# ranjanbalappa-nykaa/recommendations

Measured on AMD Instinct MI355X. Metric: training samples/sec (LTHM fwd+bwd) at 1/2/4/8 MI355X; embedding HBM GB/s, higher is better.
Workload: dtype bf16; 1 GPU; LTHM C2: item KShift P=1000000 D=32 K=16, 32 cat x 1000000 KShift D=32 K=8, T=128, d=256, 4 layers, H=4, 6 lookahead heads; global_batch=4096, per_gpu_batch=4096, seq_len=128, activation_checkpointing=False, distinct_batches=4, item_lookup=inline, parallelism=dp1

## Files before the change

### recommendations_amd/csrc/loss.hip

```cpp
#include "mfma.hpp"

#include <algorithm>
#include <cstdlib>

namespace lthm {

constexpr int DE = 128;

__device__ __forceinline__ int swz(int row) {
  const int h = (row >> 3) & 1;
  return ((((row & 7) << 1) + (h << 3)) & 15) | h;
}
__device__ __forceinline__ int ks_off256(int row, int ch) { return row * 256 + ((ch ^ swz(row)) << 4); }

template <typename TX>
__global__ __launch_bounds__(256) void rownorm_k(const TX* __restrict__ x, int64_t rows, int D, bf16_t* __restrict__ out,
                                                 float* __restrict__ norms, const uint8_t* __restrict__ mask,
                                                 int64_t mgroup, int64_t mstride) {
  const int lane = threadIdx.x & 63;
  for (int64_t r = (int64_t)blockIdx.x * 4 + (threadIdx.x >> 6); r < rows; r += (int64_t)gridDim.x * 4) {
    float v[4];
    float ss = 0.f;
#pragma unroll
    for (int i = 0; i < 4; ++i) {
// ... 1565 lines not shown
      v2 += __popcll(__ballot(ok));
    }
    if (lane == 0) { V[b] = v; V2[b] = v2; }
  }
  __syncthreads();
  const int per = (Bm + 255) / 256;
  const int r0 = min(tid * per, Bm), r1 = min(r0 + per, Bm);
  for (int pass = 0; pass < (phys ? 2 : 1); ++pass) {
    int* A = pass ? V2 : V;
    int run = 0;
    for (int b = r0; b < r1; ++b) run += A[b];
    scan[tid] = run;
    __syncthreads();
    for (int o = 1; o < 256; o <<= 1) {
      const int t = tid >= o ? scan[tid - o] : 0;
      __syncthreads();
      scan[tid] += t;
      __syncthreads();
    }
    const int total = scan[255];
    int k = scan[tid] - run;
    __syncthreads();
    for (int b = r0; b < r1; ++b) {
      const int c = A[b];
      A[b] = k;
      k += c;
    }
    if (tid == 0) A[Bm] = total;
    __syncthreads();
  }
  const int N = V[Bm];
  int* cs = a.vcs + (int64_t)mb * (a.mbs + 1);
  for (int b = tid; b <= Bm; b += 256) cs[b] = V[b];
  if (tid == 0) {
    a.vm[mb] = N;
    if (phys) a.vnp[mb] = V2[Bm];
  }
  int* cmap = a.vcmap + (int64_t)mb * a.mbs * T;
  int* pidx = a.vpidx + (int64_t)mb * a.mbs * T;
  const int L = g.L;
  for (int b = wv; b < Bm; b += 4) {
    const uint8_t* mr = mrow(b);
    int* cm = cmap + (int64_t)b * T;
    wave_compact(T, V[b], lane, [&](int tp) { return tp >= off && mr[tp] == 0; },
                 [&](int k, int tp) { a.vridx[base + k] = b * L + tp - off; cm[tp] = k; },
                 [&](int tp) { cm[tp] = -1; });
    if (phys)
      wave_compact(T, V2[b], lane, [&](int tp) { return mr[tp] == 0; },
                   [&](int k, int tp) { pidx[k] = b * T + tp; }, [&](int) {});
  }
  int u = 0;
  for (int b = tid; b < Bm; b += 256) {
    const int vb = V[b + 1] - V[b];
    u += (N - vb > 0) ? vb : 0;
  }
  const int U = (int)block_dsum((double)u, red);
  const float wr = U > 0 ? loss_scale / (float)U : 0.f;
  for (int r = tid; r < a.n_max; r += 256) {
    float wvv = 0.f;
    if (r < g.n) {
      const int b = seq_of(g, r);
      wvv = (!pad_of(a, g, r) && N - (V[b + 1] - V[b]) > 0) ? wr : 0.f;
    }
    wout[base + r] = wvv;
  }
  const int per_row = DE / 4;
  const int64_t cnt = (int64_t)Bm * (T + 1) * per_row;
  for (int64_t i = tid; i < cnt; i += 256) {
    const int row = (int)(i / per_row), c4 = (int)(i - (int64_t)row * per_row);
    const int b = row / (T + 1), t = row - b * (T + 1);
    if (t < L && mrow(b)[t + off] == 0) continue;
    const int64_t o = (((g.b0 + b) * (T + 1) + t) * a.NH + a.head) * DE + c4 * 4;
    if (a.y_dtype == LTHM_BF16) *reinterpret_cast<uint2*>(a.dy + o) = uint2{0u, 0u};
    else *reinterpret_cast<float4*>((float*)a.dy + o) = float4{0.f, 0.f, 0.f, 0.f};
  }
}

template <typename TY>
__global__ __launch_bounds__(256) void cl_vgather_k(ClArgs a0) {
  const ClArgs a = head_args(a0, blockIdx.z);
  const int mb = blockIdx.y;
  const Geo g = geo(a, mb);
  const int m = a.vm[mb];
  const int64_t base = (int64_t)mb * a.n_max;
  const int sub = threadIdx.x & 15;
  const int step = gridDim.x * 32;
  for (int i0 = blockIdx.x * 32 + (threadIdx.x >> 4); i0 < m; i0 += step) {
    int rr[2];
    u32x4 ov[2], iv[2];
    float yv[2][8];
#pragma unroll
    for (int u = 0; u < 2; ++u) rr[u] = a.vridx[base + min(i0 + 16 * u, m - 1)];
#pragma unroll
    for (int u = 0; u < 2; ++u) {
      if (a.vnorm_out) {
        const int b = rr[u] / g.L, t = rr[u] - b * g.L;
        const int64_t ro = ((g.b0 + b) * (a.T + 1) + t) * a.NH + a.head;
        ld8(reinterpret_cast<const TY*>(a.y_raw) + ro * DE + sub * 8, yv[u]);
      } else {
        ov[u] = *reinterpret_cast<const u32x4*>(out_row(a, g, rr[u]) + sub * 8);
      }
      iv[u] = *reinterpret_cast<const u32x4*>(in_row(a, g, rr[u]) + sub * 8);
    }
#pragma unroll
    for (int u = 0; u < 2; ++u) {
      const int i = i0 + 16 * u;
      if (a.vnorm_out) {
        float ss = 0.f;
#pragma unroll
        for (int k = 0; k < 8; ++k) ss += yv[u][k] * yv[u][k];
        const float nrm = sqrtf(group16_sum(ss));
        const float den = fmaxf(nrm, 1e-12f);
        float o[8];
#pragma unroll
        for (int k = 0; k < 8; ++k) o[k] = yv[u][k] / den;
        ov[u] = u32x4{pack_bf16x2(o[0], o[1]), pack_bf16x2(o[2], o[3]), pack_bf16x2(o[4], o[5]), pack_bf16x2(o[6], o[7])};
        if (i < m && sub == 0) {
          const int b = rr[u] / g.L, t = rr[u] - b * g.L;
          a.vnorm_out[((g.b0 + b) * (a.T + 1) + t) * a.NH + a.head] = nrm;
        }
      }
      float acc = 0.f;
#pragma unroll
      for (int k = 0; k < 4; ++k) {
        acc = fmaf(__uint_as_float(ov[u][k] << 16), __uint_as_float(iv[u][k] << 16), acc);
        acc = fmaf(__uint_as_float(ov[u][k] & 0xffff0000u), __uint_as_float(iv[u][k] & 0xffff0000u), acc);
      }
#pragma unroll
      for (int o = 1; o < 16; o <<= 1) acc += __shfl_xor(acc, o, 64);
      if (i < m) {
        *reinterpret_cast<u32x4*>(a.vR + (base + i) * DE + sub * 8) = ov[u];
        *reinterpret_cast<u32x4*>(a.vC + (base + i) * DE + sub * 8) = iv[u];
        if (sub == 0) a.diag[base + rr[u]] = acc / a.tau;
      }
    }
  }
}

__global__ __launch_bounds__(256) void cl_vshift_k(ClArgs a0) {
  const ClArgs a = head_args(a0, blockIdx.z);
  const int mb = blockIdx.y;
  const int m = a.vm[mb];
  const int64_t base = (int64_t)mb * a.n_max;
  for (int i = blockIdx.x * 256 + threadIdx.x; i < m; i += gridDim.x * 256) {
    const int r = a.vridx[base + i];
    const float wv = a.w[base + r];
    a.vsh[base + i] = wv != 0.f ? __log2f(wv) - a.lse[base + r] * LOG2E : -INFINITY;
    a.vw[base + i] = wv;
  }
  if (blockIdx.z != 0) return;
  const Geo g = geo(a, mb);
  const int T = a.T;
  const int per_row = DE / 4;
  const int64_t cnt = (int64_t)g.Bm * T * per_row;
  for (int64_t i = (int64_t)blockIdx.x * 256 + threadIdx.x; i < cnt; i += (int64_t)gridDim.x * 256) {
    const int row = (int)(i / per_row), c4 = (int)(i - (int64_t)row * per_row);
    const int b = row / T, t = row - b * T;
    if (a.mask[(g.b0 + b) * a.mask_stride + t] == 0) continue;
    const int64_t o = ((g.b0 + b) * T + t) * DE + c4 * 4;
    if (a.t_dtype == LTHM_BF16) *reinterpret_cast<uint2*>((bf16_t*)a.dt + o) = uint2{0u, 0u};
    else *reinterpret_cast<float4*>((float*)a.dt + o) = float4{0.f, 0.f, 0.f, 0.f};
  }
}

struct VTile {
  union {
    unsigned char img[CL_NB32][64 * 256];
    float ep[4][32][CL_EPS];
  };
};

struct VCursor {
  const unsigned char* base;
  int row0, lim, ch0;
  __device__ __forceinline__ void init(const bf16_t* base_, int lim_, int w, int lane) {
    base = reinterpret_cast<const unsigned char*>(base_);
    row0 = 16 * w + (lane >> 4);
    lim = lim_;
    ch0 = (lane & 15) ^ (((lane >> 4) & 3) << 2);
  }
  __device__ __forceinline__ void stage(unsigned char* img, int t, int w, int lane) {
#pragma unroll
    for (int k = 0; k < 4; ++k) {
      const int row = 64 * t + row0 + 4 * k;
      const void* src = row < lim ? (const void*)(base + (int64_t)row * 256 + ((ch0 ^ k) << 4))
                                  : (const void*)(cl_zero_row + 16 * (lane & 15));
      glds16(src, img + (16 * w + 4 * k) * 256);
    }
  }
};

struct TileOrder {
  int ts_lo, nspan, nclean, tl, rot;
  __device__ __forceinline__ void init(int spec_lo, int spec_hi, int m, int ntile, bool last_special) {
    ts_lo = spec_lo / 64;
    const int ts_hi = (spec_hi - 1) / 64;
    nspan = ts_hi - ts_lo + 1;
    tl = (last_special && (m & 63) && ntile - 1 > ts_hi) ? ntile - 1 : -1;
    nclean = ntile - nspan - (tl >= 0 ? 1 : 0);
    rot = 0;
  }
  __device__ __forceinline__ int at(int i) const {
    if (i < nclean && rot) {
      i += rot % nclean;
      if (i >= nclean) i -= nclean;
    }
    if (i < ts_lo) return i;
    if (i < nclean) return i + nspan;
    const int j = i - nclean;
    return j < nspan ? ts_lo + j : tl;
  }
};

__device__ __forceinline__ void s_tile32(f32x16 (&acc)[2], const unsigned char* img, const int (&roff)[8],
                                         const bf16x8v (&qf)[8]) {
  acc[0] = f32x16{};
  acc[1] = f32x16{};
  auto rd = [&](int ib, int s) {
    return frag_at(img + ib * 8192 + roff[s]);
  };
  bf16x8v f0 = rd(0, 0), f1 = rd(1, 0);
#pragma unroll
  for (int s = 0; s < 8; ++s) {
    const int sn = s + 1 < 8 ? s + 1 : s;
    const bf16x8v n0 = rd(0, sn), n1 = rd(1, sn);
    acc[0] = mfma32(f0, qf[s], acc[0]);
    acc[1] = mfma32(f1, qf[s], acc[1]);
    f0 = n0;
    f1 = n1;
  }
}

__device__ __forceinline__ void pv_tile32(f32x16 (&dacc)[4], const f32x16& p, int ib, const unsigned char* img,
                                          const int (&toff)[4][2]) {
  const bf16x8v af0 = pack_frag(p, 0), af1 = pack_frag(p, 8);
  const int k0 = 2 * ib * 4096, k1 = (2 * ib + 1) * 4096;
#pragma unroll
  for (int nd = 0; nd < 4; ++nd) {
    dacc[nd] = mfma32(af0, tr_frag32(img, toff[nd][0] + k0, toff[nd][1] + k0), dacc[nd]);
    dacc[nd] = mfma32(af1, tr_frag32(img, toff[nd][0] + k1, toff[nd][1] + k1), dacc[nd]);
  }
}

__global__ __launch_bounds__(256, 2) void cl_fr32v_k(ClArgs a0) {
  constexpr int NW = 4, XR = 32 * NW;
  __shared__ __attribute__((aligned(16))) VTile sh;
  __shared__ float rs_sc[NW][32], rs_w[NW][32], rs_pd[NW][32];
  int z = blockIdx.z, mb = blockIdx.y, xb = blockIdx.x;
  if (a0.xcd_order & 1) {
    const int per = gridDim.x * gridDim.y;
    const int lin = xcd_remap(blockIdx.x + gridDim.x * (blockIdx.y + gridDim.y * blockIdx.z), per * gridDim.z);
    z = lin / per;
    const int bid = lin - z * per;
    mb = bid / gridDim.x;
    xb = bid - mb * gridDim.x;
  }
  const ClArgs a = head_args(a0, z);
  const int m = a.vm[mb];
  const int x0 = xb * XR;
  if (x0 >= m) return;
  const Geo g = geo(a, mb);
  const int tid = threadIdx.x, lane = tid & 63, w = __builtin_amdgcn_readfirstlane(tid >> 6);
  const int r32 = lane & 31, hh = lane >> 5;
  const int64_t base = (int64_t)mb * a.n_max;
  const int* cs = a.vcs + (int64_t)mb * (a.mbs + 1);
  const int* ridx = a.vridx + base;
  int roff[8], toff[4][2];
  frag32_offsets(roff, toff, lane);
  f32x16 dacc[4];
#pragma unroll
  for (int nd = 0; nd < 4; ++nd) dacc[nd] = f32x16{};
  const int x = x0 + 32 * w + r32;
  const bool live = x < m;
  const int r = live ? ridx[x] : 0;
  bf16x8v qf[8];
  {
    const bf16_t* rp = a.vR + (base + (live ? x : 0)) * DE;
#pragma unroll
    for (int s = 0; s < 8; ++s) {
      u32x4 v = {0u, 0u, 0u, 0u};
      if (live) v = *reinterpret_cast<const u32x4*>(rp + 16 * s + 8 * hh);
      qf[s] = __builtin_bit_cast(bf16x8v, v);
    }
  }
  const float it = 1.f / a.tau, c1 = it * LOG2E, csh = -c1;
  const float dg = live ? a.diag[base + r] : 0.f;
  const float thr = rank_threshold(dg, it, a.tau);
  const int xsq = live ? seq_of(g, r) : 0;
  const int xlo = live ? cs[xsq] : -(1 << 30);
  const unsigned xlen = live ? (unsigned)(cs[xsq + 1] - cs[xsq]) : 0u;
  const int rlo = ridx[x0], rhi = ridx[min(x0 + XR, m) - 1];
  const int spec_lo = cs[seq_of(g, rlo)], spec_hi = cs[seq_of(g, rhi) + 1];
  float Z = 0.f;
  int cn = 0, rk = 0;
  const int ntile = (m + 63) / 64;
  TileOrder ord;
  ord.init(spec_lo, spec_hi, m, ntile, true);
  if (a0.xcd_order & 2) ord.rot = xb;
  VCursor cur;
  cur.init(a.vC + base * DE, m, w, lane);
  retire_loads();
  cur.stage(sh.img[0], ord.at(0), w, lane);
  if (ntile > 1) cur.stage(sh.img[1], ord.at(1), w, lane);
  if (ntile > 2) cur.stage(sh.img[2], ord.at(2), w, lane);
  if (ntile > 2) wait_vm<8>();
  else if (ntile > 1) wait_vm<4>();
  else wait_vm<0>();
  __builtin_amdgcn_s_barrier();
  f32x16 sacc[2];
  s_tile32(sacc, sh.img[0], roff, qf);
  auto open_step = [&](int i) {
    if (i + 2 < ntile) wait_vm<4>();
    else wait_vm<0>();
    __builtin_amdgcn_s_barrier();
    if (i + 3 < ntile) cur.stage(sh.img[(i + 3) % CL_NB32], ord.at(i + 3), w, lane);
  };
  for (int i = 0; i < ord.nclean; ++i) {
    open_step(i);
    const unsigned char* img = sh.img[i % CL_NB32];
    const unsigned char* imgn = sh.img[(i + 1) % CL_NB32];
#pragma unroll
    for (int ib = 0; ib < 2; ++ib) {
#pragma unroll
      for (int v = 0; v < 16; ++v) {
        const float sv = sacc[ib][v];
        const float p = __builtin_amdgcn_exp2f(__builtin_fmaf(sv, c1, csh));
        Z += p;
        rk += sv > thr ? 1 : 0;
        sacc[ib][v] = p;
      }
    }
    cn += 32;
    f32x16 snext[2];
    s_tile32(snext, imgn, roff, qf);
    pv_tile32(dacc, sacc[0], 0, img, toff);
    pv_tile32(dacc, sacc[1], 1, img, toff);
    sacc[0] = snext[0];
    sacc[1] = snext[1];
  }
  auto below = [](int k) { return k >= 64 ? ~0ull : (1ull << k) - 1ull; };
  for (int i = ord.nclean; i < ntile; ++i) {
    open_step(i);
    const unsigned char* img = sh.img[i % CL_NB32];
    const unsigned char* imgn = sh.img[(i + 1) % CL_NB32];
    const int y0 = 64 * ord.at(i);
    const int lo = min(max(xlo - y0, 0), 64), hi = min(max(xlo + (int)xlen - y0, 0), 64);
    const int me = min(max(m - y0, 0), 64);
    uint64_t keep = live ? (below(lo) | (below(me) & ~below(hi))) : 0ull;
    keep >>= 4 * hh;
    const uint32_t kw[2] = {(uint32_t)keep, (uint32_t)(keep >> 32)};
    cn += __popc(kw[0] & 0x0F0F0F0Fu) + __popc(kw[1] & 0x0F0F0F0Fu);
#pragma unroll
    for (int ib = 0; ib < 2; ++ib) {
#pragma unroll
      for (int v = 0; v < 16; ++v) {
        const int msk = __builtin_amdgcn_sbfe((int)kw[ib], 8 * (v >> 2) + (v & 3), 1);
        const float sv = __uint_as_float((__float_as_uint(sacc[ib][v]) & msk) | (0xff800000u & ~msk));
        const float p = __builtin_amdgcn_exp2f(__builtin_fmaf(sv, c1, csh));
        Z += p;
        rk += sv > thr ? 1 : 0;
        sacc[ib][v] = p;
      }
    }
    f32x16 snext[2];
    s_tile32(snext, imgn, roff, qf);
    pv_tile32(dacc, sacc[0], 0, img, toff);
    pv_tile32(dacc, sacc[1], 1, img, toff);
    sacc[0] = snext[0];
    sacc[1] = snext[1];
  }
  Z += __shfl_xor(Z, 32, 64);
  cn += __shfl_xor(cn, 32, 64);
  rk += __shfl_xor(rk, 32, 64);
  const float pd = live ? __builtin_amdgcn_exp2f((dg - it) * LOG2E) : 0.f;
  Z += pd;
  cn += live ? 1 : 0;
  const float wx = live ? a.w[base + r] : 0.f;
  if (hh == 0) {
    if (live) {
      a.lse[base + r] = it + __logf(Z);
      a.pos[base + r] = dg;
      a.cnt[base + r] = cn;
      a.rank[base + r] = rk;
    }
    rs_sc[w][r32] = (wx != 0.f && Z > 0.f) ? wx / Z : 0.f;
    rs_w[w][r32] = wx;
    rs_pd[w][r32] = pd;
  }
  __syncthreads();
#pragma unroll
  for (int nd = 0; nd < 4; ++nd)
#pragma unroll
    for (int v = 0; v < 16; ++v) sh.ep[w][8 * (v >> 2) + 4 * hh + (v & 3)][32 * nd + r32] = dacc[nd][v];
  __syncthreads();
  const float gs = 1.f / a.tau;
  const int sub = lane & 15;
#pragma unroll 1
  for (int ps = 0; ps < 8; ++ps) {
    const int rl = 4 * ps + (lane >> 4), xr = x0 + 32 * w + rl;
    const int xc = min(xr, m - 1);
    const int rr = ridx[xc];
    const int b = rr / g.L, t = rr - b * g.L;
    const int64_t ro = ((g.b0 + b) * (a.T + 1) + t) * a.NH + a.head;
    const float sc = rs_sc[w][rl], wr = rs_w[w][rl], pdr = rs_pd[w][rl];
    float inv[8];
    load_vec<bf16_t, 16>(a.vC + (base + xc) * DE + 8 * sub, inv);
    const float4 u0 = *reinterpret_cast<const float4*>(&sh.ep[w][rl][8 * sub]);
    const float4 u1 = *reinterpret_cast<const float4*>(&sh.ep[w][rl][8 * sub + 4]);
    const float uu[8] = {u0.x, u0.y, u0.z, u0.w, u1.x, u1.y, u1.z, u1.w};
    float gv[8];
#pragma unroll
    for (int i = 0; i < 8; ++i) gv[i] = gs * (__builtin_fmaf(pdr, inv[i], uu[i]) * sc - wr * inv[i]);
    normalize_bwd_store(gv, a.y_raw, a.y_dtype, a.y_norm[ro], a.dy, ro * DE + 8 * sub, xr < m);
  }
}

__global__ __launch_bounds__(256, 2) void cl_bwd32v_k(ClArgs a0) {
  constexpr int NW = 4, XR = 32 * NW;
  __shared__ __attribute__((aligned(16))) ClTile32<NW> sh;
  const int per = gridDim.x * gridDim.y;
  const int lin = xcd_remap(blockIdx.x + gridDim.x * blockIdx.y, per);
  const int mb = lin / gridDim.x, xb = lin - mb * gridDim.x;
  const int tid = threadIdx.x, lane = tid & 63, w = __builtin_amdgcn_readfirstlane(tid >> 6);
  const int r32 = lane & 31, hh = lane >> 5;
  const int T = a0.T;
  const int64_t b0 = (int64_t)mb * a0.mbs;
  const int np = a0.vnp[mb];
  const int j0 = xb * XR;
  if (j0 >= np) return;
  const int* pidx = a0.vpidx + (int64_t)mb * a0.mbs * T;
  const int j = j0 + 32 * w + r32;
  const bool pin = j < np;
  const int p = pidx[pin ? j : np - 1];
  const int pb = p / T, pt = p - pb * T;
  int roff[8], toff[4][2];
  frag32_offsets(roff, toff, lane);
  f32x16 dacc[4];
#pragma unroll
  for (int nd = 0; nd < 4; ++nd) dacc[nd] = f32x16{};
  bf16x8v qf[8];
  {
    const bf16_t* rp = a0.in_n + ((b0 + pb) * T + pt) * DE;
#pragma unroll
    for (int s = 0; s < 8; ++s) {
      u32x4 v = {0u, 0u, 0u, 0u};
      if (pin) v = *reinterpret_cast<const u32x4*>(rp + 16 * s + 8 * hh);
      qf[s] = __builtin_bit_cast(bf16x8v, v);
    }
  }
  const int b_lo = pidx[j0] / T, b_hi = pidx[min(j0 + XR, np) - 1] / T;
  const float c1 = LOG2E / a0.tau;
  const int nrun = a0.heads_run;
#pragma unroll 1
  for (int hz = 0; hz < nrun; ++hz) {
    const ClArgs a = head_args(a0, hz);
    const int m = a.vm[mb];
    if (m == 0) continue;
    const int64_t base = (int64_t)mb * a.n_max;
    const int* cs = a.vcs + (int64_t)mb * (a.mbs + 1);
    const int xc = pin ? a.vcmap[(int64_t)mb * a.mbs * T + p] : -1;
    const bool live = xc >= 0;
    const int xlo = cs[pb];
    const unsigned xlen = (unsigned)(cs[pb + 1] - xlo);
    const int spec_lo = cs[b_lo], spec_hi = cs[b_hi + 1];
    const bool wmask = __ballot(!live) != 0ull;
    const float* shv = a.vsh + base;
    const float* wvv = a.vw + base;
    VCursor cur;
    cur.init(a.vR + base * DE, m, w, lane);
    const int ntile = (m + 63) / 64;
    TileOrder ord;
    ord.init(spec_lo, spec_hi, m, ntile, false);
    auto stage = [&](int i) {
      const int buf = i % CL_NB32, y0 = ord.at(i) * 64;
      cur.stage(sh.r.img[buf], ord.at(i), w, lane);
      const bool inr = y0 + lane < m;
      glds4(inr ? shv + y0 + lane : &cl_ninf, sh.r.m0[buf][w]);
      glds4(inr ? wvv + y0 + lane : &cl_zero_f, sh.r.m1[buf][w]);
    };
    constexpr int PT = 6;
    __syncthreads();
    retire_loads();
    stage(0);
    if (ntile > 1) stage(1);
    if (ntile > 2) stage(2);
    auto open_step = [&](int i) {
      if (i + 2 < ntile) wait_vm<2 * PT>();
      else if (i + 1 < ntile) wait_vm<PT>();
      else wait_vm<0>();
      __builtin_amdgcn_s_barrier();
      if (i + 3 < ntile) stage(i + 3);
    };
    for (int i = 0; i < ord.nclean; ++i) {
      open_step(i);
      const int cb = i % CL_NB32;
      const unsigned char* img = sh.r.img[cb];
      f32x16 acc[2];
      s_tile32(acc, img, roff, qf);
#pragma unroll
      for (int ib = 0; ib < 2; ++ib)
#pragma unroll
        for (int qd = 0; qd < 4; ++qd) {
          const float4 ys = *reinterpret_cast<const float4*>(&sh.r.m0[cb][w][32 * ib + 8 * qd + 4 * hh]);
          const float yv[4] = {ys.x, ys.y, ys.z, ys.w};
#pragma unroll
          for (int jj = 0; jj < 4; ++jj)
            acc[ib][4 * qd + jj] = __builtin_amdgcn_exp2f(__builtin_fmaf(acc[ib][4 * qd + jj], c1, yv[jj]));
        }
      if (wmask && !live) {
        acc[0] = f32x16{};
        acc[1] = f32x16{};
      }
      pv_tile32(dacc, acc[0], 0, img, toff);
      pv_tile32(dacc, acc[1], 1, img, toff);
    }
    for (int i = ord.nclean; i < ntile; ++i) {
      open_step(i);
      const int cb = i % CL_NB32;
      const unsigned char* img = sh.r.img[cb];
      f32x16 acc[2];
      s_tile32(acc, img, roff, qf);
      const int y0 = 64 * ord.at(i);
      const int lo = min(max(xlo - y0, 0), 64), hi = min(max(xlo + (int)xlen - y0, 0), 64);
      auto below = [](int k) { return k >= 64 ? ~0ull : (1ull << k) - 1ull; };
      const int dd = xc - y0;
      uint64_t keep = below(lo) | ~below(hi);
      if (live && dd >= 0 && dd < 64) keep |= 1ull << dd;
      keep >>= 4 * hh;
      const uint32_t kw[2] = {(uint32_t)keep, (uint32_t)(keep >> 32)};
      int dx = dd - 4 * hh;
      asm volatile("" : "+v"(dx));
#pragma unroll
      for (int ib = 0; ib < 2; ++ib)
#pragma unroll
        for (int qd = 0; qd < 4; ++qd) {
          const float4 ys = *reinterpret_cast<const float4*>(&sh.r.m0[cb][w][32 * ib + 8 * qd + 4 * hh]);
          const float4 ws = *reinterpret_cast<const float4*>(&sh.r.m1[cb][w][32 * ib + 8 * qd + 4 * hh]);
          const float yv[4] = {ys.x, ys.y, ys.z, ys.w}, wv4[4] = {ws.x, ws.y, ws.z, ws.w};
#pragma unroll
          for (int jj = 0; jj < 4; ++jj) {
            const int v = 4 * qd + jj, cv = 8 * qd + jj;
            const int msk = __builtin_amdgcn_sbfe((int)kw[ib], cv, 1);
            const float sv = __uint_as_float((__float_as_uint(acc[ib][v]) & msk) | (0xff800000u & ~msk));
            const float e = __builtin_amdgcn_exp2f(__builtin_fmaf(sv, c1, yv[jj]));
            const uint32_t dm = 0u - (uint32_t)(dx == 32 * ib + cv);
            acc[ib][v] = e - __uint_as_float(__float_as_uint(wv4[jj]) & dm);
          }
        }
      if (wmask && !live) {
        acc[0] = f32x16{};
        acc[1] = f32x16{};
      }
      pv_tile32(dacc, acc[0], 0, img, toff);
      pv_tile32(dacc, acc[1], 1, img, toff);
    }
  }
  __syncthreads();
#pragma unroll
  for (int nd = 0; nd < 4; ++nd)
#pragma unroll
    for (int v = 0; v < 16; ++v) sh.ep[w][8 * (v >> 2) + 4 * hh + (v & 3)][32 * nd + r32] = dacc[nd][v];
  const float gs = (a0.gscale ? *a0.gscale : 1.f) / a0.tau;
  const int sub = lane & 15;
#pragma unroll 1
  for (int ps = 0; ps < 8; ++ps) {
    const int rl = 4 * ps + (lane >> 4), q = j0 + 32 * w + rl;
    const int pq = pidx[min(q, np - 1)];
    const int64_t ro = b0 * T + pq;
    float gv[8];
    const float4 u0 = *reinterpret_cast<const float4*>(&sh.ep[w][rl][8 * sub]);
    const float4 u1 = *reinterpret_cast<const float4*>(&sh.ep[w][rl][8 * sub + 4]);
    gv[0] = gs * u0.x; gv[1] = gs * u0.y; gv[2] = gs * u0.z; gv[3] = gs * u0.w;
    gv[4] = gs * u1.x; gv[5] = gs * u1.y; gv[6] = gs * u1.z; gv[7] = gs * u1.w;
    normalize_bwd_store(gv, a0.t_raw, a0.t_dtype, a0.t_norm[ro], a0.dt, ro * DE + 8 * sub, q < np);
  }
}

}

using namespace lthm;

static ClArgs cl_args(const lthm_contrastive_desc* d) {
  ClArgs a;
  a.out_n = (const bf16_t*)d->out_n; a.in_n = (const bf16_t*)d->in_n; a.mask = d->mask; a.mask_stride = d->mask_stride;
  a.B = d->B; a.T = d->T; a.NH = d->n_heads; a.head = d->head; a.mbs = d->mb_size; a.n_mb = d->n_mb; a.n_max = d->n_max;
  a.offsets = d->offsets; a.tau = d->tau;
  a.lse = d->lse; a.pos = d->pos; a.cnt = d->cnt; a.rank = d->rank; a.diag = d->diag; a.w = d->w;
  a.gscale = d->gscale;
  a.d_out = d->d_out; a.d_in = d->d_in;
  a.colb = nullptr;
  a.lq = d->logq; a.lq_stride = d->logq_stride; a.lqcol = d->logq_col;
  a.y_raw = (const bf16_t*)d->y_raw; a.y_norm = d->y_norm; a.dy = (bf16_t*)d->dy;
  a.head_stride = d->head_stride;
  a.y_dtype = d->y_dtype;
  a.heads_run = d->heads_run > 1 ? d->heads_run : 1;
  a.t_raw = d->t_raw; a.t_dtype = d->t_dtype; a.t_norm = d->t_norm; a.dt = d->dt;
  a.xcd_order = 0;
  a.vm = nullptr; a.vcs = nullptr; a.vridx = nullptr; a.vsh = nullptr; a.vw = nullptr; a.vcmap = nullptr;
  a.vR = nullptr; a.vC = nullptr; a.vpidx = nullptr; a.vnp = nullptr; a.vnorm_out = nullptr;
  if (d->vc_ws) {
    const VcLayout L = vc_layout(d->n_heads, d->n_mb, d->mb_size, d->T, d->n_max);
    char* b = (char*)d->vc_ws;
    a.vm = (int*)(b + L.m); a.vnp = (int*)(b + L.np); a.vcs = (int*)(b + L.cs); a.vridx = (int*)(b + L.ridx);
    a.vsh = (float*)(b + L.sh); a.vw = (float*)(b + L.w); a.vcmap = (int*)(b + L.cmap); a.vpidx = (int*)(b + L.pidx);
    a.vR = (bf16_t*)(b + L.R); a.vC = (bf16_t*)(b + L.C);
  }
  return a;
}

static int cl_check(const lthm_contrastive_desc* d) {
  if (!d || d->De != DE || d->B <= 0 || d->T <= 0 || d->mb_size <= 0 || d->n_mb <= 0) return 1;
  if ((int64_t)d->mb_size * d->T > d->n_max || d->n_max % 64 != 0) return 1;
  if ((int64_t)d->n_max * d->T >= (1ll << 32)) return 1;
  if (d->head < 0 || d->head >= d->n_heads) return 1;
  if (d->logq && (!d->logq_col || d->logq_stride < d->T)) return 1;
  return 0;
}

static int64_t cl_stats_blocks(int32_t n_max) { return (n_max + CL_SROWS - 1) / CL_SROWS; }

extern "C" int64_t lthm_contrastive_vc_ws_bytes(int64_t B, int32_t T, int32_t n_heads, int32_t mb_size, int32_t n_mb,
                                                int32_t n_max) {
  if (B <= 0 || T <= 0 || n_heads <= 0 || mb_size <= 0 || n_mb <= 0 || n_max <= 0) return -1;
  return vc_layout(n_heads, n_mb, mb_size, T, n_max).total;
}

static bool vc_ok(const lthm_contrastive_desc* d) {
  if (!d->vc_ws) return false;
  if (!d->out_n && !(d->y_raw && d->y_norm)) return false;
  if (d->vc_ws_bytes < vc_layout(d->n_heads, d->n_mb, d->mb_size, d->T, d->n_max).total) return false;
  return d->head == 0 && d->heads_run == d->n_heads && d->head_stride == (int64_t)d->n_mb * d->n_max &&
         d->mb_size <= CL_UMAXB && (int64_t)d->mb_size * d->T <= (1ll << 30);
}

extern "C" int64_t lthm_contrastive_ws_bytes(int32_t n_mb, int32_t n_max, int32_t heads) {
  if (n_mb <= 0 || n_max <= 0 || heads <= 0) return -1;
  const int64_t hm = (int64_t)heads * n_mb;
  return hm * n_max * 4 + ((hm * n_max * 4) % 8) + hm * cl_stats_blocks(n_max) * CL_NPART * 8;
}

template <typename TX>
static void launch_rownorm(const TX* x, int64_t rows, int D, bf16_t* out, float* norms, const uint8_t* mask,
                           int64_t mgroup, int64_t mstride, hipStream_t s) {
  if (D % 8 == 0) {
    const int grid = grid_for(rows, 16, 256 * 8);
    if (D <= 128)
      hipLaunchKernelGGL((rownorm_v8_k<TX, 1>), dim3(grid), dim3(256), 0, s, x, rows, D, out, norms, mask, mgroup, mstride);
    else
      hipLaunchKernelGGL((rownorm_v8_k<TX, 2>), dim3(grid), dim3(256), 0, s, x, rows, D, out, norms, mask, mgroup, mstride);
  } else {
    hipLaunchKernelGGL((rownorm_k<TX>), dim3(grid_for(rows, 4, 256 * 8)), dim3(256), 0, s, x, rows, D, out, norms,
                       mask, mgroup, mstride);
  }
}

template <typename TX>
static void launch_rownorm_bwd(const TX* x, const float* norms, const float* g, int64_t rows, int D, bf16_t* dx_bf,
                               float* dx_f, hipStream_t s) {
  if (D % 8 == 0) {
    const int grid = grid_for(rows, 16, 256 * 8);
    if (D <= 128)
      hipLaunchKernelGGL((rownorm_bwd_v8_k<TX, 1>), dim3(grid), dim3(256), 0, s, x, norms, g, rows, D, dx_bf, dx_f);
    else
      hipLaunchKernelGGL((rownorm_bwd_v8_k<TX, 2>), dim3(grid), dim3(256), 0, s, x, norms, g, rows, D, dx_bf, dx_f);
  } else {
    hipLaunchKernelGGL((rownorm_bwd_k<TX>), dim3(grid_for(rows, 4, 256 * 8)), dim3(256), 0, s, x, norms, g, rows, D,
                       dx_bf, dx_f);
  }
}

extern "C" int lthm_rownorm(const void* x, int32_t x_dtype, int64_t rows, int32_t D, void* out_bf16, float* norms,
                            const uint8_t* row_mask, int64_t mask_group, int64_t mask_stride, void* stream) {
// ... 176 lines not shown
```

Baseline: 109,000 samples/s.

## Process two score tiles per barrier in the loss kernel pipeline

```diff
diff --git a/recommendations_amd/csrc/loss.hip b/recommendations_amd/csrc/loss.hip
--- a/recommendations_amd/csrc/loss.hip
+++ b/recommendations_amd/csrc/loss.hip
@@ -1891,23 +1891,13 @@
   retire_loads();
   cur.stage(sh.img[0], ord.at(0), w, lane);
   if (ntile > 1) cur.stage(sh.img[1], ord.at(1), w, lane);
-  if (ntile > 2) cur.stage(sh.img[2], ord.at(2), w, lane);
-  if (ntile > 2) wait_vm<8>();
-  else if (ntile > 1) wait_vm<4>();
-  else wait_vm<0>();
-  __builtin_amdgcn_s_barrier();
-  f32x16 sacc[2];
-  s_tile32(sacc, sh.img[0], roff, qf);
   auto open_step = [&](int i) {
-    if (i + 2 < ntile) wait_vm<4>();
-    else wait_vm<0>();
+    wait_vm<0>();
     __builtin_amdgcn_s_barrier();
+    if (i + 2 < ntile) cur.stage(sh.img[(i + 2) % CL_NB32], ord.at(i + 2), w, lane);
     if (i + 3 < ntile) cur.stage(sh.img[(i + 3) % CL_NB32], ord.at(i + 3), w, lane);
   };
-  for (int i = 0; i < ord.nclean; ++i) {
-    open_step(i);
-    const unsigned char* img = sh.img[i % CL_NB32];
-    const unsigned char* imgn = sh.img[(i + 1) % CL_NB32];
+  auto elems_clean = [&](f32x16 (&sacc)[2]) {
 #pragma unroll
     for (int ib = 0; ib < 2; ++ib) {
 #pragma unroll
@@ -1920,18 +1910,9 @@
       }
     }
     cn += 32;
-    f32x16 snext[2];
-    s_tile32(snext, imgn, roff, qf);
-    pv_tile32(dacc, sacc[0], 0, img, toff);
-    pv_tile32(dacc, sacc[1], 1, img, toff);
-    sacc[0] = snext[0];
-    sacc[1] = snext[1];
-  }
+  };
   auto below = [](int k) { return k >= 64 ? ~0ull : (1ull << k) - 1ull; };
-  for (int i = ord.nclean; i < ntile; ++i) {
-    open_step(i);
-    const unsigned char* img = sh.img[i % CL_NB32];
-    const unsigned char* imgn = sh.img[(i + 1) % CL_NB32];
+  auto elems_special = [&](f32x16 (&sacc)[2], int i) {
     const int y0 = 64 * ord.at(i);
     const int lo = min(max(xlo - y0, 0), 64), hi = min(max(xlo + (int)xlen - y0, 0), 64);
     const int me = min(max(m - y0, 0), 64);
@@ -1951,12 +1932,38 @@
         sacc[ib][v] = p;
       }
     }
-    f32x16 snext[2];
-    s_tile32(snext, imgn, roff, qf);
-    pv_tile32(dacc, sacc[0], 0, img, toff);
-    pv_tile32(dacc, sacc[1], 1, img, toff);
-    sacc[0] = snext[0];
-    sacc[1] = snext[1];
+  };
+  int ti = 0;
+  for (; ti + 1 < ord.nclean; ti += 2) {
+    open_step(ti);
+    const unsigned char* img0 = sh.img[ti % CL_NB32];
+    const unsigned char* img1 = sh.img[(ti + 1) % CL_NB32];
+    f32x16 s0[2], s1[2];
+    s_tile32(s0, img0, roff, qf);
+    __builtin_amdgcn_sched_barrier(0);
+    s_tile32(s1, img1, roff, qf);
+    elems_clean(s0);
+    __builtin_amdgcn_sched_barrier(0);
+    pv_tile32(dacc, s0[0], 0, img0, toff);
+    pv_tile32(dacc, s0[1], 1, img0, toff);
+    elems_clean(s1);
+    __builtin_amdgcn_sched_barrier(0);
+    pv_tile32(dacc, s1[0], 0, img1, toff);
+    pv_tile32(dacc, s1[1], 1, img1, toff);
+  }
+  auto special_tile = [&](int i) {
+    const unsigned char* img = sh.img[i % CL_NB32];
+    f32x16 s0[2];
+    s_tile32(s0, img, roff, qf);
+    elems_special(s0, i);
+    pv_tile32(dacc, s0[0], 0, img, toff);
+    pv_tile32(dacc, s0[1], 1, img, toff);
+  };
+  for (; ti < ntile; ti += 2) {
+    open_step(ti);
+    special_tile(ti);
+    __builtin_amdgcn_sched_barrier(0);
+    if (ti + 1 < ntile) special_tile(ti + 1);
   }
   Z += __shfl_xor(Z, 32, 64);
   cn += __shfl_xor(cn, 32, 64);
```

Result: no change. 109,100 samples/s (median of 2 runs) (+0.1%).
